# furio1999/EO_Diffusion

Measured on AMD Instinct MI355X. Metric: denoising steps/sec (UNet fwd + DDPM update) at 256x256 bs=16, higher is better.
Workload: dtype f32; 1 GPU; DDPM sampling step, 256x256x3, batch 16 per GPU, UNet arch A0 (base 128, mults [1,2,3,4], 1 res-block(s), attn_res []), Philox noise, x0-clipped update; global_batch=16, image_size=256, parallelism=batch-sharded x1, accumulate=fp32, precision_mode=fp32x3

## Files before the change

eo_diffusion_amd/csrc/igemm.hip:

```cpp
#include <type_traits>

#include "common.h"

struct IgemmP {
    const char* a0;
    const char* a1;
    const char* b;
    const float* bias;
    const float* cbias;
    const char* res;
    char* y;
    long long cbias_stride;
    int N, H, W, C0, C1, Cin, Cout, KS, stride, pad, ups, pad_tl, Ho, Wo, HoWo, Heff, Weff;
    int tw_log2, th;
    int tiles_pw, tiles_pi;
    long long lda, ldb, ldc, sa0, sa1, sb0, sb1, sc0, sc1;
    int nb1, bias_mode, c_f32;
    long long M;
    int Ncols, K, taps, KT, tiles_m, tiles_n, out_nchw;
    int kc0, kc1;
    int tapmajor_log2;
    int ldk;
    const float* gn_ss;
    int gn_silu;
// ... 1503 lines not shown
                for (int i = 0; i < TM; ++i)
#pragma unroll
                    for (int j = 0; j < TN; ++j)
                        acc[i][j] = DIRECT ? __builtin_amdgcn_mfma_f32_16x16x32_f16(__builtin_bit_cast(half8, bl[j]), __builtin_bit_cast(half8, ah[i]), acc[i][j], 0, 0, 0)
                                           : __builtin_amdgcn_mfma_f32_16x16x32_f16(__builtin_bit_cast(half8, ah[i]), __builtin_bit_cast(half8, bl[j]), acc[i][j], 0, 0, 0);
#pragma unroll
                for (int i = 0; i < TM; ++i)
#pragma unroll
                    for (int j = 0; j < TN; ++j)
                        acc[i][j] = DIRECT ? __builtin_amdgcn_mfma_f32_16x16x32_f16(__builtin_bit_cast(half8, bh[j]), __builtin_bit_cast(half8, ah[i]), acc[i][j], 0, 0, 0)
                                           : __builtin_amdgcn_mfma_f32_16x16x32_f16(__builtin_bit_cast(half8, ah[i]), __builtin_bit_cast(half8, bh[j]), acc[i][j], 0, 0, 0);
            } else {
#pragma unroll
                for (int s2 = 0; s2 < 2; ++s2) {
                    const int o = ((4 * s2 + lh) ^ bsw) * 16;
                    i32x4 fa16[TM], fb16[TN];
#pragma unroll
                    for (int i = 0; i < TM; ++i) fa16[i] = *reinterpret_cast<const i32x4*>(stg + a_rd + i * MS * BKB + o);
#pragma unroll
                    for (int j = 0; j < TN; ++j) fb16[j] = *reinterpret_cast<const i32x4*>(stg + b_rd2 + j * MS * BKB + o);
#pragma unroll
                    for (int i = 0; i < TM; ++i)
#pragma unroll
                        for (int j = 0; j < TN; ++j)
                            acc[i][j] = __builtin_amdgcn_mfma_f32_16x16x32_f16(__builtin_bit_cast(half8, fa16[i]), __builtin_bit_cast(half8, fb16[j]), acc[i][j], 0, 0, 0);
                }
            }
        }
      }
    }
    __builtin_amdgcn_s_waitcnt(0xc07f);
    __builtin_amdgcn_s_barrier();
    EOD_STAMP_AT(2);
    IgemmP pe = p;
    if constexpr (KSPLIT) pe.y = p.y + (long long)blockIdx.y * p.M * p.Cout * 4;
    if constexpr (SPLIT) {
        pe.alpha = p.alpha * wsc1 * asc.inv;
        if constexpr (DIRECT) halo_epilogue_direct<BM, BN, WAVES_M, WAVES_N>(pe, g, acc, wave, lane, n0, pre_bq, pe.alpha, pre_we);
        else igemm_epilogue<T, true, BM, BN, WAVES_M, WAVES_N, true, MS>(pe, g, acc, smem, wave, lane, n0, nullptr, 0, pre_bcol);
    } else if constexpr (sizeof(T) == 2) {
        igemm_epilogue<T, true, BM, BN, WAVES_M, WAVES_N, KSPLIT, MS>(pe, g, acc, smem, wave, lane, n0, nullptr, 0, pre_bcol);
    } else {
        igemm_epilogue<T, true, BM, BN, WAVES_M, WAVES_N, sizeof(T) == 4, MS>(pe, g, acc, smem, wave, lane, n0, nullptr, 0, pre_bcol);
    }
    }
    EOD_STAMP_AT(3);
}

template <typename T, bool SPLIT, bool BWD = false>
__global__ __launch_bounds__(256, 2) void conv_up4_halo_kernel(const IgemmP p) {
    static_assert(!SPLIT || sizeof(T) == 4, "the split-fp16 product is a mode of fp32 storage");
    static_assert(SPLIT || sizeof(T) == 2, "fp16 storage or split fp32");
    constexpr int NW = 4, WAVES_M = 2, WAVES_N = 2, BN = 128, BM = 128, MS = 16;
    constexpr int PH = 10, PW = 18, PR = PH * PW, PG = (PR + 7) / 8, LAH = (PG + NW - 1) / NW;
    constexpr int ES = sizeof(T), EPC = 16 / ES, BKB = 128, BK = BKB / ES;
    constexpr int WM = BM / WAVES_M, WN = BN / WAVES_N, TM = WM / MS, TN = WN / MS;
    constexpr int LB = (BN / 8) / NW;
    constexpr int ABUF = PG * 1024, BSTAGE = BN * BKB;
    static_assert(LAH == 6, "schedule: three patch pieces per K-step in steps 0 and 1");

    extern __shared__ __attribute__((aligned(16))) char smem[];
    char* const sA = smem;
    char* const sB = smem + 2 * ABUF;

    constexpr bool DIRECT = SPLIT && !BWD;
    const int tid = threadIdx.x, lane = tid & 63;
    const int wave = __builtin_amdgcn_readfirstlane(tid >> 6);
    const int wm = wave / WAVES_N, wn = wave % WAVES_N;
    int tile_m, tile_nn;
    map_tile(p, tile_m, tile_nn);
    const int tpc = BWD ? p.tiles_n : p.tiles_n >> 2;
    const int cls = BWD ? 0 : tile_nn / tpc, n0 = (tile_nn - cls * tpc) * BN;
    const int par_y = cls >> 1, par_x = cls & 1;
    const TileGeom g = make_geom<true, BM>(p, tile_m);
    float pre_bcol[DIRECT ? 1 : TN];
    f32x4 pre_bq[DIRECT ? TN : 1];
    int pre_we[DIRECT ? TN : 1];
    if constexpr (DIRECT) {
        prefetch_bcol4<TN>(p, p.Cout, n0 + wn * WN, lane, g.n_first, pre_bq);
        prefetch_wexp4<TN>(p, p.Cout, n0 + wn * WN, cls * p.Cout, lane, pre_we);
    } else {
        prefetch_bcol<TN, MS>(p, p.Cout, n0 + wn * WN, lane, g.n_first, pre_bcol);
    }
    float wsc1 = 1.0f;
    if constexpr (SPLIT) wsc1 = p.w_scale[1];
    AbScale asc = {EOD_SPLIT_ASCALE, 1.0f};
    if constexpr (SPLIT) {
        if (p.a_bound) asc = ab_scale_of(ab_wave_bound(p.a_bound, g.n_first));
    }

    const int srow = lane >> 3, sslot = lane & 7;
    unsigned ppix[LAH];
    const int bchunk0 = sslot ^ ((4 * wave + (srow >> 1)) & 7);
    unsigned pck = 0, pvalid = 0;
#pragma unroll
    for (int i = 0; i < LAH; ++i) {
        const int prow = (wave + NW * i) * 8 + srow;
        const int py = prow / PW, px = prow - py * PW;
        const int hi = g.ty0 - 1 + py, wi = g.tx0 - 1 + px;
        const bool ok = (wave + NW * i) < PG && prow < PR && (unsigned)hi < (unsigned)p.H && (unsigned)wi < (unsigned)p.W;
        if (ok) pvalid |= 1u << i;
        ppix[i] = BWD ? (unsigned)(4 * hi * p.W + 2 * wi)
                      : (unsigned)(hi * p.W + wi);
        pck |= (unsigned)(sslot ^ ((px >> 1) & 7)) << (3 * i);
    }
    auto pchunk_of = [&](int i) { return (int)((pck >> (3 * i)) & 7u); };
    unsigned b_v[LB];
#pragma unroll
    for (int i = 0; i < LB; ++i) {
        const int row = (wave + NW * i) * 8 + srow;
        b_v[i] = (n0 + row < p.Cout) ? (unsigned)(row * (BWD ? 4 * p.C0 : p.Cin) * ES) + bchunk0 * 16 : EOD_OOB;
    }
    const __amdgpu_buffer_rsrc_t rsA = make_rsrc(p.a0 + (long long)g.n_first * p.H * p.W * p.C0 * ES * (BWD ? 4 : 1));
    const int bpitch = BWD ? 4 * p.C0 : p.Cin;
    const __amdgpu_buffer_rsrc_t rsB = make_rsrc(p.b + ((long long)cls * p.Cout + n0) * bpitch * ES);
    const int tapstride = (BWD ? p.Cout * bpitch : 4 * p.Cout * p.Cin) * ES;

    struct Chunk {
        int kin, cls;
        bool ktail;
    };
    auto chunk_of = [&](int cc) {
        Chunk c;
        c.cls = BWD ? (cc & 3) : cls;
        c.kin = (BWD ? (cc >> 2) : cc) * BK;
        c.ktail = c.kin + BK > p.C0;
        return c;
    };
    auto issue_patch_piece = [&](int i, const Chunk& c, char* abuf) {
        const int pc = pchunk_of(i);
        unsigned v = ((pvalid >> i) & 1u) ? ppix[i] * (unsigned)(p.C0 * ES) + pc * 16 : EOD_OOB;
        if (c.ktail) v = (c.kin + pc * EPC < p.C0) ? v : EOD_OOB;
        const unsigned soff = (unsigned)(c.kin * ES) + (BWD ? (unsigned)(((c.cls >> 1) * 2 * p.W + (c.cls & 1)) * p.C0 * ES) : 0u);
        blds16(rsA, v, soff, abuf + (wave + NW * i) * 1024);
    };
    auto split_piece = [&](int i, char* abuf) {
        char* ptr = abuf + (wave + NW * i) * 1024 + lane * 16;
        const f32x4 f = *reinterpret_cast<const f32x4*>(ptr);
        *reinterpret_cast<i32x4*>(ptr) = split_pair_exchange_scaled(f, asc.s, (pchunk_of(i) & 1) != 0);
    };
    auto issue_weights = [&](int s, const Chunk& c, char* bst) {
        const int oy = BWD ? 1 - (c.cls >> 1) : par_y, ox = BWD ? 1 - (c.cls & 1) : par_x;
        const int tap = (oy + (s & 1)) * 3 + ox + (s >> 1);
        const unsigned soff = (unsigned)(tap * tapstride) + (unsigned)((c.kin + (BWD ? c.cls * p.C0 : 0)) * ES);
#pragma unroll
        for (int i = 0; i < LB; ++i) {
            unsigned v = b_v[i];
            if (c.ktail) v = (c.kin + (SPLIT ? (bchunk0 >> 1) * 8 : bchunk0 * EPC) < p.C0) ? v : EOD_OOB;
            blds16(rsB, v, soff, bst + (wave + NW * i) * 1024);
        }
    };
    auto wait_vm = [](int n) {
        switch (n) {
            case 0: asm volatile("s_waitcnt vmcnt(0)" ::: "memory"); break;
            case 1: asm volatile("s_waitcnt vmcnt(1)" ::: "memory"); break;
            case 2: asm volatile("s_waitcnt vmcnt(2)" ::: "memory"); break;
            case 3: asm volatile("s_waitcnt vmcnt(3)" ::: "memory"); break;
            case 4: asm volatile("s_waitcnt vmcnt(4)" ::: "memory"); break;
            case 5: asm volatile("s_waitcnt vmcnt(5)" ::: "memory"); break;
            default: asm volatile("s_waitcnt vmcnt(6)" ::: "memory"); break;
        }
    };

    typename AccLayout<MS>::vec acc[TM][TN];
#pragma unroll
    for (int i = 0; i < TM; ++i)
#pragma unroll
        for (int j = 0; j < TN; ++j)
#pragma unroll
            for (int r = 0; r < AccLayout<MS>::R; ++r) acc[i][j][r] = 0.0f;

    const int lr = lane & 15, lh = lane >> 4;
    const int c0 = SPLIT ? 2 * ((0x2130 >> (4 * lh)) & 3) : lh, c1 = SPLIT ? c0 + 1 : 4 + lh;
    int acur[2][2];
    auto set_acur = [&](int oy, int ox, int aoff) {
#pragma unroll
        for (int b = 0; b < 2; ++b) {
            const int pxc = lr + ox + b;
            const int key = (pxc >> 1) & 7;
            const int rowb = ((wm * (WM / 16) + oy) * PW + pxc) * BKB + aoff;
            acur[0][b] = rowb + ((c0 ^ key) << 4);
            acur[1][b] = rowb + ((c1 ^ key) << 4);
        }
    };
    set_acur(BWD ? 1 : par_y, BWD ? 1 : par_x, 0);
    const int bsw = (lr >> 1) & 7;
    const int b_rd = (wn * WN + lr) * BKB;
    const int boff0 = b_rd + ((c0 ^ bsw) << 4), boff1 = b_rd + ((c1 ^ bsw) << 4);

    i32x4 aw[2][TM];
    auto a_load = [&](int v, int b, int a) {
#pragma unroll
        for (int r = 0; r < TM + 1; ++r)
            if (a == 0 ? r < TM : r == TM) aw[v][r % TM] = *reinterpret_cast<const i32x4*>(sA + acur[v][b] + r * PW * BKB);
    };
    const int KC = BWD ? 4 * p.kc0 : p.kc0, NSTEP = KC * 4;
    {
        const Chunk ch0 = chunk_of(0);
#pragma unroll
        for (int i = 0; i < LAH; ++i)
            if ((wave + NW * i) < PG) issue_patch_piece(i, ch0, sA);
        issue_weights(0, ch0, sB);
        if constexpr (SPLIT) {
            asm volatile("s_waitcnt vmcnt(0)" ::: "memory");
#pragma unroll
            for (int i = 0; i < LAH; ++i)
                if ((wave + NW * i) < PG) split_piece(i, sA);
        }
    }
    int np_prev = 0;
    int step = 0;
    for (int cc = 0; cc < KC; ++cc) {
        const Chunk cur = chunk_of(cc);
        const bool has_next = cc + 1 < KC;
        const Chunk nxt = chunk_of(has_next ? cc + 1 : cc);
        char* abuf_next = sA + ((cc + 1) & 1) * ABUF;
#pragma unroll
        for (int s = 0; s < 4; ++s, ++step) {
            wait_vm(np_prev);
            if constexpr (SPLIT) __builtin_amdgcn_s_waitcnt(0xc07f);
            __builtin_amdgcn_s_barrier();
            const bool w_next = step + 1 < NSTEP;
            if (w_next) issue_weights((s + 1) & 3, s == 3 ? nxt : cur, sB + ((step + 1) & 1) * BSTAGE);
            int np = 0;
            if (s < 2 && has_next) {
#pragma unroll
                for (int k = 0; k < 3; ++k)
                    if ((wave + NW * (3 * s + k)) < PG) {
                        issue_patch_piece(3 * s + k, nxt, abuf_next);
                        ++np;
                    }
            }
            const int a = s & 1, b = s >> 1;
            const char* bst = sB + (step & 1) * BSTAGE;
            if constexpr (SPLIT) {
                i32x4 bh[TN], bl[TN];
                a_load(1, b, a);
#pragma unroll
                for (int j = 0; j < TN; ++j) bh[j] = *reinterpret_cast<const i32x4*>(bst + boff0 + j * MS * BKB);
                a_load(0, b, a);
#pragma unroll
                for (int i = 0; i < TM; ++i)
#pragma unroll
                    for (int j = 0; j < TN; ++j)
                        acc[i][j] = DIRECT ? __builtin_amdgcn_mfma_f32_16x16x32_f16(__builtin_bit_cast(half8, bh[j]), __builtin_bit_cast(half8, aw[1][(i + a) % TM]), acc[i][j], 0, 0, 0)
                                           : __builtin_amdgcn_mfma_f32_16x16x32_f16(__builtin_bit_cast(half8, aw[1][(i + a) % TM]), __builtin_bit_cast(half8, bh[j]), acc[i][j], 0, 0, 0);
#pragma unroll
                for (int j = 0; j < TN; ++j) bl[j] = *reinterpret_cast<const i32x4*>(bst + boff1 + j * MS * BKB);
#pragma unroll
                for (int i = 0; i < TM; ++i)
#pragma unroll
                    for (int j = 0; j < TN; ++j)
                        acc[i][j] = DIRECT ? __builtin_amdgcn_mfma_f32_16x16x32_f16(__builtin_bit_cast(half8, bl[j]), __builtin_bit_cast(half8, aw[0][(i + a) % TM]), acc[i][j], 0, 0, 0)
                                           : __builtin_amdgcn_mfma_f32_16x16x32_f16(__builtin_bit_cast(half8, aw[0][(i + a) % TM]), __builtin_bit_cast(half8, bl[j]), acc[i][j], 0, 0, 0);
#pragma unroll
                for (int i = 0; i < TM; ++i)
#pragma unroll
                    for (int j = 0; j < TN; ++j)
                        acc[i][j] = DIRECT ? __builtin_amdgcn_mfma_f32_16x16x32_f16(__builtin_bit_cast(half8, bh[j]), __builtin_bit_cast(half8, aw[0][(i + a) % TM]), acc[i][j], 0, 0, 0)
                                           : __builtin_amdgcn_mfma_f32_16x16x32_f16(__builtin_bit_cast(half8, aw[0][(i + a) % TM]), __builtin_bit_cast(half8, bh[j]), acc[i][j], 0, 0, 0);
            } else {
#pragma unroll
                for (int v = 0; v < 2; ++v) {
                    i32x4 fb16[TN];
                    a_load(v, b, a);
#pragma unroll
                    for (int j = 0; j < TN; ++j) fb16[j] = *reinterpret_cast<const i32x4*>(bst + (v ? boff1 : boff0) + j * MS * BKB);
#pragma unroll
                    for (int i = 0; i < TM; ++i)
#pragma unroll
                        for (int j = 0; j < TN; ++j)
                            acc[i][j] = __builtin_amdgcn_mfma_f32_16x16x32_f16(__builtin_bit_cast(half8, aw[v][(i + a) % TM]), __builtin_bit_cast(half8, fb16[j]), acc[i][j], 0, 0, 0);
                }
            }
            if constexpr (SPLIT) {
                if (s >= 2 && has_next) {
#pragma unroll
                    for (int k = 0; k < 3; ++k)
                        if ((wave + NW * (3 * (s - 2) + k)) < PG) split_piece(3 * (s - 2) + k, abuf_next);
                }
            }
            np_prev = np;
        }
        if constexpr (BWD) {
            const int ncl = (cc + 1) & 3;
            set_acur(1 - (ncl >> 1), 1 - (ncl & 1), ((cc + 1) & 1) * ABUF);
        } else {
            const int flip = (cc & 1) ? -ABUF : ABUF;
#pragma unroll
            for (int b = 0; b < 2; ++b) {
                acur[0][b] += flip;
                acur[1][b] += flip;
            }
        }
    }
    __builtin_amdgcn_s_waitcnt(0xc07f);
    __builtin_amdgcn_s_barrier();
    IgemmP pe = p;
    pe.Ncols = p.Cout;
    TileGeom ge = g;
    if constexpr (!BWD) {
        pe.par = 1; pe.par_y = par_y; pe.par_x = par_x;
        pe.Wd = p.W;
        pe.tiles_per_image = p.tiles_pi * 4;
        ge.tile_m = g.n_first * pe.tiles_per_image + (tile_m - g.n_first * p.tiles_pi) * 4 + cls;
    }
    if constexpr (SPLIT) pe.alpha = p.alpha * wsc1 * asc.inv;
    if constexpr (!BWD) pe.w_row0 = cls * p.Cout;
    if constexpr (DIRECT) halo_epilogue_direct<BM, BN, WAVES_M, WAVES_N>(pe, ge, acc, wave, lane, n0, pre_bq, pe.alpha, pre_we);
    else igemm_epilogue<T, true, BM, BN, WAVES_M, WAVES_N, sizeof(T) == 4, MS>(pe, ge, acc, smem, wave, lane, n0, nullptr, 0, pre_bcol);
}

template <typename T, bool SPLIT, bool BWD = false> static int launch_up4(IgemmP& p, hipStream_t st) {
    constexpr int BK = 128 / (int)sizeof(T);
    const size_t ring = 2 * (size_t)(23 * 1024) + 2 * (size_t)128 * 128;
    const size_t epi = 4 * (size_t)64 * (64 + 4) * sizeof(float);
    const size_t lds = ring > epi ? ring : epi;
    auto kern = conv_up4_halo_kernel<T, SPLIT, BWD>;
    static bool attr_done = false;
    if (!attr_done) {
        (void)hipFuncSetAttribute(reinterpret_cast<const void*>(kern), hipFuncAttributeMaxDynamicSharedMemorySize, (int)lds);
        attr_done = true;
    }
    p.kc0 = (p.C0 + BK - 1) / BK;
    p.kc1 = 0;
    p.KT = p.kc0 * 4;
    p.tiles_n = (BWD ? 1 : 4) * ((p.Cout + 127) / 128);
    p.tw_log2 = 4;
    p.th = 8;
    p.tiles_pw = (p.W + 15) / 16;
    p.tiles_pi = p.tiles_pw * (p.H / 8);
    p.tiles_m = p.tiles_pi * p.N;
    const long long nblk = (long long)p.tiles_m * p.tiles_n;
    if (nblk <= 0 || nblk > 0x7fffffffLL) {
        eod_set_error("conv_up4: bad grid %lld", nblk);
        return EOD_EINVAL;
    }
    hipLaunchKernelGGL(kern, dim3((unsigned)nblk), dim3(256), lds, st, p);
    EOD_CHECK_LAUNCH("conv_up4_halo");
    return EOD_OK;
}

template <typename T, bool SPLIT>
__global__ __launch_bounds__(256, 2) void conv_s2_halo_kernel(const IgemmP p) {
    static_assert(!SPLIT || sizeof(T) == 4, "the split-fp16 product is a mode of fp32 storage");
    static_assert(SPLIT || sizeof(T) == 2, "fp16 storage or split fp32");
    constexpr int NW = 4, WAVES_M = 2, WAVES_N = 2, BN = 128, BM = 128, MS = 16;
    constexpr int PH = 9, PW = 17, PR = PH * PW, PG = (PR + 7) / 8, LAH = (PG + NW - 1) / NW;
    constexpr int ES = sizeof(T), EPC = 16 / ES, BKB = 128, BK = BKB / ES;
    constexpr int WM = BM / WAVES_M, WN = BN / WAVES_N, TM = WM / MS, TN = WN / MS;
    constexpr int LB = (BN / 8) / NW;
    constexpr int ABUF = PG * 1024, BSTAGE = BN * BKB;
    static_assert(PG == NW * LAH && LAH * 4 <= 32, "every wave stages LAH whole pieces; 4 plane-validity bits per piece");
    static_assert(LB <= 6, "wait_vm immediates");

    extern __shared__ __attribute__((aligned(16))) char smem[];
    char* const sA = smem;
    char* const sB = smem + 2 * ABUF;

    constexpr bool DIRECT = SPLIT;
    const int tid = threadIdx.x, lane = tid & 63;
    const int wave = __builtin_amdgcn_readfirstlane(tid >> 6);
    const int wm = wave / WAVES_N, wn = wave % WAVES_N;
    int tile_m, tile_n;
    map_tile(p, tile_m, tile_n);
    const int n0 = tile_n * BN;
    const TileGeom g = make_geom<true, BM>(p, tile_m);
    float pre_bcol[DIRECT ? 1 : TN];
    f32x4 pre_bq[DIRECT ? TN : 1];
    int pre_we[DIRECT ? TN : 1];
    if constexpr (DIRECT) {
        prefetch_bcol4<TN>(p, p.Cout, n0 + wn * WN, lane, g.n_first, pre_bq);
        prefetch_wexp4<TN>(p, p.Cout, n0 + wn * WN, 0, lane, pre_we);
    } else {
        prefetch_bcol<TN, MS>(p, p.Cout, n0 + wn * WN, lane, g.n_first, pre_bcol);
    }
    float wsc1 = 1.0f;
    if constexpr (SPLIT) wsc1 = p.w_scale[1];
    AbScale asc = {EOD_SPLIT_ASCALE, 1.0f};
    if constexpr (SPLIT) {
        if (p.a_bound) asc = ab_scale_of(ab_wave_bound(p.a_bound, g.n_first));
    }

    const int srow = lane >> 3, sslot = lane & 7;
    int ppix[LAH];
    unsigned pvalid = 0, pck = 0;
    const int bchunk0 = sslot ^ ((4 * wave + (srow >> 1)) & 7);
#pragma unroll
    for (int i = 0; i < LAH; ++i) {
        const int prow = (wave + NW * i) * 8 + srow;
        const int py = prow / PW, px = prow - py * PW;
        const int hi = 2 * (g.ty0 + py) - 1, wi = 2 * (g.tx0 + px) - 1;
// ... 929 lines not shown
    if (tiles <= 0 || tiles >= 128 || kt < 8) return 1;
    int s = (int)(512 / tiles);
    if (s > kt / 4) s = kt / 4;
    if (s > 16) s = 16;
    return s < 2 ? 1 : s;
}

enum { FAM_UP4, FAM_UP4_BWD, FAM_FIRST, FAM_S2_HALO, FAM_HEAD, FAM_HALO, FAM_GENERIC, FAM_GENERIC_PARITY };
struct ConvPlan {
    int Heff, Weff, Ho, Wo;
    bool halo;
    int family;
    int bn;
    bool plus128;
    bool direct;
    int splitk, splitk_per;
    int tpw;
    int64_t workspace_bytes;
    int stats_slots;
    bool gn_fusable, skip_ok;
};
static ConvPlan conv_plan(const eod_conv_desc* d) {
    ConvPlan pl = {};
    pl.bn = 128;
    pl.splitk = pl.tpw = 1;
    if (d->upsample == 4) {
        pl.family = FAM_UP4_BWD;
        pl.Heff = pl.Ho = d->H / 2;
        pl.Weff = pl.Wo = d->W / 2;
        return pl;
    }
    pl.Heff = d->H * (d->upsample ? 2 : 1);
    pl.Weff = d->W * (d->upsample ? 2 : 1);
    const int Ho = pl.Ho = conv_out_hw(d, pl.Heff), Wo = pl.Wo = conv_out_hw(d, pl.Weff);
    const bool split = d->w_split, exact = !split && d->dtype != EOD_F16, gn = d->gn_scale_shift, skip = d->skip_x;
    pl.halo = conv_uses_halo(d, Ho, Wo);
    pl.splitk = conv_splitk(d, Ho, Wo, pl.halo, opt(OPT_HALO_SPLITK) != 0, &pl.splitk_per);
    pl.workspace_bytes = pl.splitk > 1 ? (int64_t)pl.splitk * d->N * Ho * Wo * d->Cout * 4 : 0;

    if (d->out_nchw_f32 || d->Cout % (16 / eod_esize(d->dtype))) pl.stats_slots = 0;
    else if (d->upsample == 3) pl.stats_slots = (d->H / 8) * ((d->W + 15) / 16) * 8;
    else if (pl.splitk > 1) pl.stats_slots = 1;
    else if (pl.halo) pl.stats_slots = (Ho / 8) * ((Wo + 15) / 16) * 2;
    else if ((Ho * Wo) % 128 != 0) pl.stats_slots = 0;
    else pl.stats_slots = (Ho * Wo / 128) * (d->Cout > 64 ? 2 : 4);

    const int max_cout = opt(OPT_GN_FUSE_MAX_COUT) >= 0 ? opt(OPT_GN_FUSE_MAX_COUT) : (split ? 512 : 256);
    pl.gn_fusable = !d->upsample && d->Cout <= max_cout && pl.halo;
    pl.skip_ok = opt(OPT_SKIP_FUSE) != 0 && conv_skip_geom_ok(d) && pl.halo;

    const long long tiles_pi = (long long)(Ho / 8) * ((Wo + 15) / 16);
    if (d->upsample == 3) {
        pl.family = FAM_UP4;
    } else if (opt(OPT_FIRST) != 0 && conv_first_ok(d, Ho, Wo)) {
        pl.family = FAM_FIRST;
    } else if (opt(OPT_S2_HALO) != 0 && conv_s2_halo_ok(d, Ho, Wo) && pl.splitk <= 1) {
        pl.family = FAM_S2_HALO;
    } else if (opt(OPT_HEAD) != 0 && pl.halo && conv_head_ok(d)) {
        pl.family = FAM_HEAD;
        int tpw = opt(OPT_HEAD_TPW);
        if (tpw <= 0) {
            tpw = 16;
            while (tpw > 1 && (tiles_pi % tpw || tiles_pi * d->N / tpw < 512)) tpw >>= 1;
        }
        while (tpw > 1 && tiles_pi % tpw) --tpw;
        pl.tpw = tpw;
    } else if (pl.halo) {
        pl.family = FAM_HALO;
        const bool on256 = opt(OPT_HALO_BN256) != 0;
        if (d->Cout <= 32) {
            pl.bn = 32;
        } else if (d->upsample || pl.splitk > 1) {
            pl.bn = 128;
        } else if (!exact && 16 * tiles_pi * ((d->Cout + 127) / 128) < 256) {
            pl.bn = 64;
        } else if (on256 && d->Cout % 256 == 0 && d->N * tiles_pi * (d->Cout / 256) >= 256 && ((gn && !exact) || (split && skip))) {
            pl.bn = 256;
        } else if (on256 && d->Cout > 256 && d->Cout % 256 == 128 && d->N * tiles_pi * ((d->Cout - 128) / 256) >= 256 && split && gn) {
            pl.bn = 256;
            pl.plus128 = true;
        }
    } else {
        pl.family = pl.splitk <= 1 && !split && conv_parity_ok(d, Ho, Wo) ? FAM_GENERIC_PARITY : FAM_GENERIC;
        pl.bn = generic_bn(d->Cout);
        if (split && d->Cout > 64) {
            const long long M = (long long)d->N * Ho * Wo;
            if (d->Cout % 256 == 0 && pl.splitk <= 1 && ((M + 127) / 128) * (d->Cout / 256) >= 256 && opt(OPT_HALO_BN256)) pl.bn = 256;
            pl.direct = pl.splitk <= 1 && !d->out_nchw_f32 && (Ho * Wo) % 128 == 0 && M % 128 == 0 && d->Cout % 4 == 0;
        }
    }
    return pl;
}

extern "C" int eod_conv_skip_ok(const eod_conv_desc* d) { return d && conv_plan(d).skip_ok ? 1 : 0; }
extern "C" int eod_conv_gn_fusable(const eod_conv_desc* d) { return d && conv_plan(d).gn_fusable ? 1 : 0; }
extern "C" int64_t eod_conv_workspace_size(const eod_conv_desc* d) { return d ? conv_plan(d).workspace_bytes : 0; }
extern "C" int eod_conv_stats_slots(const eod_conv_desc* d) { return d ? conv_plan(d).stats_slots : 0; }
extern "C" const char* eod_conv_kernel_name(const eod_conv_desc* d) {
    if (!d) return "";
    const ConvPlan pl = conv_plan(d);
    switch (pl.family) {
        case FAM_UP4: case FAM_UP4_BWD: return "conv_up4_halo_kernel";
        case FAM_FIRST: return "conv_first_x3_kernel";
        case FAM_S2_HALO: return "conv_s2_halo_kernel";
        case FAM_HEAD: return "conv_head_kernel";
        case FAM_HALO: return pl.bn == 32 ? "conv3x3_halo_kernel<BN=32>" : "conv3x3_halo_kernel";
        default: return "igemm_kernel";
    }
}

extern "C" int eod_conv_halo_columns(const eod_conv_desc* d) {
    if (!d) return 0;
    const ConvPlan pl = conv_plan(d);
    return pl.family == FAM_HALO ? pl.bn : 0;
}

static int conv_up4_bwd(const eod_conv_desc* d, void* stream) {
    EOD_REQUIRE(d->N > 0 && d->H > 0 && d->W > 0 && d->C0 > 0 && d->Cout > 0 && d->x && d->w && d->y, "conv (upsample 4): bad args");
    EOD_REQUIRE(conv_up4_bwd_ok(d), "conv: upsample = 4 needs a geometry for which eod_conv_up4_bwd_ok(d) == 1");
    EOD_REQUIRE(eod_aligned16(d->x) && eod_aligned16(d->w), "conv: 16-byte alignment");
    EOD_REQUIRE((long long)d->H * d->W * d->C0 * 2 < 0x7fffffffLL && 9LL * d->Cout * 4 * d->C0 * 2 < 0x7fffffffLL, "conv (upsample 4): operand exceeds the 2 GiB window");
    const ConvPlan pl = conv_plan(d);
    IgemmP p = {};
    p.a0 = (const char*)d->x; p.b = (const char*)d->w; p.bias = d->bias; p.bias_mode = d->bias ? 1 : 0;
    p.cbias = d->cbias; p.cbias_stride = d->cbias_stride; p.res = (const char*)d->res; p.y = (char*)d->y;
    p.N = d->N; p.H = pl.Ho; p.W = pl.Wo;
    p.C0 = d->C0; p.C1 = 0; p.Cin = d->C0; p.Cout = d->Cout; p.KS = 3; p.stride = 1; p.pad = 1;
    p.Ho = pl.Ho; p.Wo = pl.Wo; p.HoWo = pl.Ho * pl.Wo; p.Heff = pl.Heff; p.Weff = pl.Weff;
    p.Hd = pl.Ho; p.Wd = pl.Wo; p.HWd = pl.Ho * pl.Wo;
    p.M = (long long)d->N * pl.Ho * pl.Wo; p.Ncols = d->Cout; p.taps = 9; p.alpha = d->alpha; p.nb1 = 1; p.tapmajor_log2 = -1;
    return launch_up4<half_t, false, true>(p, (hipStream_t)stream);
}

static IgemmP splitk_partial(const IgemmP& p, const eod_conv_desc* d, const ConvPlan& pl) {
    IgemmP q = p;
    q.stats = nullptr;
    q.splitk = pl.splitk;
    q.splitk_per = pl.splitk_per;
    q.y = (char*)d->workspace;
    q.bias = nullptr; q.bias_mode = 0; q.cbias = nullptr; q.res = nullptr; q.alpha = 1.0f;
    return q;
}
static int splitk_finish(const eod_conv_desc* d, const IgemmP& p, int splitk, hipStream_t st) {
    if (d->stats) {
        const dim3 grid((unsigned)((p.Cout + 63) / 64), (unsigned)d->N);
        if (d->dtype == EOD_F16)
            hipLaunchKernelGGL(splitk_reduce_stats_kernel<half_t>, grid, dim3(256), 0, st, (const float*)d->workspace, splitk, p.M, p.Cout, p.HoWo, d->alpha, d->bias, d->cbias, (long long)d->cbias_stride, (const half_t*)d->res, (half_t*)d->y, d->stats);
        else
            hipLaunchKernelGGL(splitk_reduce_stats_kernel<float>, grid, dim3(256), 0, st, (const float*)d->workspace, splitk, p.M, p.Cout, p.HoWo, d->alpha, d->bias, d->cbias, (long long)d->cbias_stride, (const float*)d->res, (float*)d->y, d->stats);
        EOD_CHECK_LAUNCH("splitk_reduce_stats");
        return EOD_OK;
    }
    const long long total4 = p.M * p.Cout / 4;
    const unsigned blocks = (unsigned)((total4 + 255) / 256 > 2048 ? 2048 : (total4 + 255) / 256);
    if (d->dtype == EOD_F16)
        hipLaunchKernelGGL(splitk_reduce_kernel<half_t>, dim3(blocks), dim3(256), 0, st, (const float*)d->workspace, splitk, p.M, p.Cout, p.HoWo, d->alpha, d->bias, d->cbias, (long long)d->cbias_stride, (const half_t*)d->res, (half_t*)d->y, (const float*)nullptr);
    else
        hipLaunchKernelGGL(splitk_reduce_kernel<float>, dim3(blocks), dim3(256), 0, st, (const float*)d->workspace, splitk, p.M, p.Cout, p.HoWo, d->alpha, d->bias, d->cbias, (long long)d->cbias_stride, (const float*)d->res, (float*)d->y, (const float*)nullptr);
    EOD_CHECK_LAUNCH("splitk_reduce");
    return EOD_OK;
}
static int conv_require_workspace(const eod_conv_desc* d, const ConvPlan& pl) {
    EOD_REQUIRE(d->workspace && d->workspace_bytes >= pl.workspace_bytes, "conv: workspace of %lld bytes required (eod_conv_workspace_size)", (long long)pl.workspace_bytes);
    return EOD_OK;
}

template <typename T, bool SPLIT, int MS, bool GN, bool SKIP>
// ... 55 lines not shown
    IgemmP p = {};
    p.a0 = (const char*)d->x;
    p.a1 = (const char*)d->x2;
    p.b = (const char*)d->w;
    p.bias = d->bias;
    p.bias_mode = d->bias ? 1 : 0;
    p.cbias = d->cbias;
    p.cbias_stride = d->cbias_stride;
    p.res = (const char*)d->res;
    p.y = (char*)d->y;
    p.N = d->N; p.H = d->H; p.W = d->W; p.C0 = d->C0; p.C1 = d->C1; p.Cin = d->C0 + d->C1; p.Cout = d->Cout;
    p.KS = d->ksize; p.stride = d->stride; p.pad = d->pad; p.ups = d->upsample; p.pad_tl = d->pad_tl;
    p.Ho = Ho; p.Wo = Wo; p.HoWo = Ho * Wo; p.Heff = pl.Heff; p.Weff = pl.Weff;
    p.Hd = Ho; p.Wd = Wo; p.HWd = Ho * Wo;
    p.M = (long long)d->N * Ho * Wo;
    p.Ncols = d->Cout;
    p.taps = d->ksize * d->ksize;
    p.out_nchw = d->out_nchw_f32;
    p.alpha = d->alpha;
    p.nb1 = 1;
    p.tapmajor_log2 = -1;
    if (d->w_tapmajor) {
        const int cpt = d->C0 / epc;
        EOD_REQUIRE(d->ksize == 3 && d->C1 == 0 && !d->upsample && !d->pad_tl && !d->gn_scale_shift && (cpt == 1 || cpt == 2 || cpt == 4),
                    "conv: w_tapmajor needs a 3x3 conv of a single source with C0 in {1,2,4} x %d channels", epc);
        p.tapmajor_log2 = cpt == 1 ? 0 : cpt == 2 ? 1 : 2;
        p.ldk = eod_conv_tapmajor_ldk(d->C0, d->dtype);
    }
    hipStream_t st = (hipStream_t)stream;
    if (d->stats) {
        EOD_REQUIRE(pl.stats_slots > 0 && pl.stats_slots == d->stats_slots, "conv: stats_slots=%d but this geometry provides %d", d->stats_slots, pl.stats_slots);
        p.stats = d->stats;
        p.stats_P = pl.stats_slots;
        p.tiles_per_image = Ho * Wo / 128;
    }
    EOD_REQUIRE(!d->w_split || (conv_split_ok(d) && d->w_scale),
                "conv: w_split needs a geometry for which eod_conv_split_ok(d) == 1 and the w_scale of eod_pack_conv_weight_split");
    p.w_scale = d->w_split ? d->w_scale : nullptr;
    p.w_rexp = d->w_split ? reinterpret_cast<const int*>(d->w_scale) + 4 : nullptr;
    p.w_row0 = 0;
    p.a_bound = d->w_split ? d->a_bound : nullptr;
    EOD_REQUIRE(!d->x_presplit || (d->w_split && d->a_bound && !pl.halo && !d->upsample && !d->w_tapmajor && !d->gn_scale_shift),
                "conv: x_presplit needs w_split with the producer's bound table, on the generic kernel (1x1 / stride-2 / small maps)");
    p.a_ps = d->x_presplit;
    EOD_REQUIRE(!d->y_presplit_bound || (d->w_split && !pl.halo && !d->out_nchw_f32 && !d->stats && d->Cout % 8 == 0 && (Ho * Wo) % 128 == 0 &&
                                         pl.splitk <= 1),
                "conv: y_presplit_bound needs w_split on the generic kernel, Cout %% 8 == 0, whole 128-row tiles per image, no statistics");
    p.y_ps_bound = d->y_presplit_bound;
    p.skip_bound = (d->w_split && d->skip_x) ? d->skip_bound : nullptr;
    const bool f16 = d->dtype == EOD_F16;
    switch (pl.family) {
        case FAM_UP4:
            EOD_REQUIRE(conv_up4_ok(d), "conv: upsample = 3 (parity-class form of the nearest-2x conv) needs a geometry for which eod_conv_up4_ok(d) == 1");
            return f16 ? launch_up4<half_t, false>(p, st) : launch_up4<float, true>(p, st);
        case FAM_FIRST: return d->C0 == 4 ? launch_first<4>(p, st) : launch_first<8>(p, st);
        case FAM_S2_HALO: return f16 ? launch_s2<half_t, false>(p, st) : launch_s2<float, true>(p, st);
        case FAM_HEAD:
            p.gn_ss = d->gn_scale_shift;
            p.gn_silu = d->gn_silu;
            p.tpw = pl.tpw;
            return f16 ? launch_head<half_t, false>(p, st) : launch_head<float, true>(p, st);
        default: break;
    }
    const bool splitk = pl.splitk > 1;
    if (pl.family == FAM_HALO && splitk) {
        const int rc = conv_require_workspace(d, pl);
        if (rc != EOD_OK) return rc;
    }
    if (d->skip_x) {
        EOD_REQUIRE(pl.skip_ok && d->skip_w, "conv: skip_x needs a geometry for which eod_conv_skip_ok(d) == 1, and skip_w");
        EOD_REQUIRE((d->skip_C1 > 0) == (d->skip_x2 != nullptr), "conv: skip_x2 / skip_C1 mismatch");
        EOD_REQUIRE(eod_aligned16(d->skip_x) && eod_aligned16(d->skip_x2) && eod_aligned16(d->skip_w), "conv: 16-byte alignment (skip operands)");
        const long long smax = d->skip_C0 > d->skip_C1 ? d->skip_C0 : d->skip_C1;
        EOD_REQUIRE((long long)d->H * d->W * smax * es < 0x7fffffffLL && (long long)d->Cout * (d->skip_C0 + d->skip_C1) * es < 0x7fffffffLL,
                    "conv: skip operand exceeds the 2 GiB window");
        p.sx0 = (const char*)d->skip_x;
        p.sx1 = (const char*)d->skip_x2;
        p.b2 = (const char*)d->skip_w;
        p.SC0 = d->skip_C0;
        p.SC1 = d->skip_C1;
    }
    if (pl.family == FAM_HALO) {
        if (d->gn_scale_shift) {
            EOD_REQUIRE(!d->upsample, "conv: fused input GroupNorm is not available together with upsample");
            p.gn_ss = d->gn_scale_shift;
            p.gn_silu = d->gn_silu;
        }
        IgemmP q = splitk ? splitk_partial(p, d, pl) : p;
        const int rc = d->w_split ? launch_halo_T<float, true, 16>(q, d, pl, st)
                                  : f16 ? launch_halo_T<half_t, false, 16>(q, d, pl, st) : launch_halo_T<float, false, 32>(q, d, pl, st);
        return splitk && rc == EOD_OK ? splitk_finish(d, p, pl.splitk, st) : rc;
    }
    EOD_REQUIRE(!d->gn_scale_shift, "conv: fused input GroupNorm needs the halo-patch kernel (ask eod_conv_gn_fusable first)");
    if (pl.family == FAM_GENERIC_PARITY) {
        p.par = 1;
        p.Hd = Ho / 2; p.Wd = Wo / 2; p.HWd = p.Hd * p.Wd;
        p.M = (long long)d->N * p.HWd;
        for (int cls = 0; cls < 4; ++cls) {
            IgemmP q = p;
            q.par_y = cls >> 1; q.par_x = cls & 1;
            const int ndy = q.par_y ? 2 : 1, ndx = q.par_x ? 2 : 1;
            const int dys[2] = {q.par_y ? 0 : 1, 2}, dxs[2] = {q.par_x ? 0 : 1, 2};
            q.taps = 0; q.taplist = 0;
            for (int a = 0; a < ndy; ++a)
                for (int b = 0; b < ndx; ++b) q.taplist |= (unsigned)(dys[a] * 3 + dxs[b]) << (4 * q.taps++);
            const int rc = f16 ? launch_T<half_t, true>(q, 1, st) : launch_T<float, true>(q, 1, st);
// ... 57 lines not shown
```

Measured before the change: 41.79 steps/s.

## Add 8-wave BN=256 upsample conv kernel and shrink parity-class patch window

Adds an 8-wave, 256-column variant of the parity-class nearest-2x upsample conv for the split-fp16 fp32 path. It is selected when the grid stays large enough, with a 128-column remainder handled by the existing kernel through a new n_base offset. It also shrinks the staged input patch from 10x18 to 9x17 in the forward path by folding the parity offset into the load coordinates. The aim is to reuse each staged input patch across more output channels and to load less halo. The cost is higher LDS and register use at one block per CU, plus possibly two launches per conv.

After: 42.23 steps/s, median of 6. +1.1%, better.

```diff
diff --git a/eo_diffusion_amd/csrc/igemm.hip b/eo_diffusion_amd/csrc/igemm.hip
--- a/eo_diffusion_amd/csrc/igemm.hip
+++ b/eo_diffusion_amd/csrc/igemm.hip
@@ -1579,12 +1579,13 @@
     static_assert(!SPLIT || sizeof(T) == 4, "the split-fp16 product is a mode of fp32 storage");
     static_assert(SPLIT || sizeof(T) == 2, "fp16 storage or split fp32");
     constexpr int NW = 4, WAVES_M = 2, WAVES_N = 2, BN = 128, BM = 128, MS = 16;
-    constexpr int PH = 10, PW = 18, PR = PH * PW, PG = (PR + 7) / 8, LAH = (PG + NW - 1) / NW;
+    constexpr int PH = BWD ? 10 : 9, PW = BWD ? 18 : 17, PR = PH * PW, PG = (PR + 7) / 8, LAH = (PG + NW - 1) / NW;
     constexpr int ES = sizeof(T), EPC = 16 / ES, BKB = 128, BK = BKB / ES;
     constexpr int WM = BM / WAVES_M, WN = BN / WAVES_N, TM = WM / MS, TN = WN / MS;
     constexpr int LB = (BN / 8) / NW;
     constexpr int ABUF = PG * 1024, BSTAGE = BN * BKB;
-    static_assert(LAH == 6, "schedule: three patch pieces per K-step in steps 0 and 1");
+    static_assert(LAH == (BWD ? 6 : 5), "schedule: up to three patch pieces per K-step in steps 0 and 1");
+    static_assert((WAVES_M - 1) * (WM / 16) + TM + (BWD ? 1 : 0) < PH && 15 + 1 + (BWD ? 1 : 0) < PW, "the fragment reads stay inside the staged patch");
 
     extern __shared__ __attribute__((aligned(16))) char smem[];
     char* const sA = smem;
@@ -1597,7 +1598,7 @@
     int tile_m, tile_nn;
     map_tile(p, tile_m, tile_nn);
     const int tpc = BWD ? p.tiles_n : p.tiles_n >> 2;
-    const int cls = BWD ? 0 : tile_nn / tpc, n0 = (tile_nn - cls * tpc) * BN;
+    const int cls = BWD ? 0 : tile_nn / tpc, n0 = (BWD ? 0 : p.n_base) + (tile_nn - cls * tpc) * BN;
     const int par_y = cls >> 1, par_x = cls & 1;
     const TileGeom g = make_geom<true, BM>(p, tile_m);
     float pre_bcol[DIRECT ? 1 : TN];
@@ -1624,7 +1625,7 @@
     for (int i = 0; i < LAH; ++i) {
         const int prow = (wave + NW * i) * 8 + srow;
         const int py = prow / PW, px = prow - py * PW;
-        const int hi = g.ty0 - 1 + py, wi = g.tx0 - 1 + px;
+        const int hi = g.ty0 - 1 + py + (BWD ? 0 : par_y), wi = g.tx0 - 1 + px + (BWD ? 0 : par_x);
         const bool ok = (wave + NW * i) < PG && prow < PR && (unsigned)hi < (unsigned)p.H && (unsigned)wi < (unsigned)p.W;
         if (ok) pvalid |= 1u << i;
         ppix[i] = BWD ? (unsigned)(4 * hi * p.W + 2 * wi)
@@ -1710,7 +1711,7 @@
             acur[1][b] = rowb + ((c1 ^ key) << 4);
         }
     };
-    set_acur(BWD ? 1 : par_y, BWD ? 1 : par_x, 0);
+    set_acur(BWD ? 1 : 0, BWD ? 1 : 0, 0);
     const int bsw = (lr >> 1) & 7;
     const int b_rd = (wn * WN + lr) * BKB;
     const int boff0 = b_rd + ((c0 ^ bsw) << 4), boff1 = b_rd + ((c1 ^ bsw) << 4);
@@ -1753,7 +1754,7 @@
             if (s < 2 && has_next) {
 #pragma unroll
                 for (int k = 0; k < 3; ++k)
-                    if ((wave + NW * (3 * s + k)) < PG) {
+                    if (3 * s + k < LAH && (wave + NW * (3 * s + k)) < PG) {
                         issue_patch_piece(3 * s + k, nxt, abuf_next);
                         ++np;
                     }
@@ -1804,7 +1805,7 @@
                 if (s >= 2 && has_next) {
 #pragma unroll
                     for (int k = 0; k < 3; ++k)
-                        if ((wave + NW * (3 * (s - 2) + k)) < PG) split_piece(3 * (s - 2) + k, abuf_next);
+                        if (3 * (s - 2) + k < LAH && (wave + NW * (3 * (s - 2) + k)) < PG) split_piece(3 * (s - 2) + k, abuf_next);
                 }
             }
             np_prev = np;
@@ -1840,7 +1841,7 @@
 
 template <typename T, bool SPLIT, bool BWD = false> static int launch_up4(IgemmP& p, hipStream_t st) {
     constexpr int BK = 128 / (int)sizeof(T);
-    const size_t ring = 2 * (size_t)(23 * 1024) + 2 * (size_t)128 * 128;
+    const size_t ring = 2 * (size_t)((BWD ? 23 : 20) * 1024) + 2 * (size_t)128 * 128;
     const size_t epi = 4 * (size_t)64 * (64 + 4) * sizeof(float);
     const size_t lds = ring > epi ? ring : epi;
     auto kern = conv_up4_halo_kernel<T, SPLIT, BWD>;
@@ -1852,7 +1853,7 @@
     p.kc0 = (p.C0 + BK - 1) / BK;
     p.kc1 = 0;
     p.KT = p.kc0 * 4;
-    p.tiles_n = (BWD ? 1 : 4) * ((p.Cout + 127) / 128);
+    p.tiles_n = BWD ? (p.Cout + 127) / 128 : 4 * ((p.Cout - p.n_base + 127) / 128);
     p.tw_log2 = 4;
     p.th = 8;
     p.tiles_pw = (p.W + 15) / 16;
@@ -1865,6 +1866,230 @@
     }
     hipLaunchKernelGGL(kern, dim3((unsigned)nblk), dim3(256), lds, st, p);
     EOD_CHECK_LAUNCH("conv_up4_halo");
+    return EOD_OK;
+}
+
+template <typename T, bool SPLIT, bool BWD, int WAVES_N>
+__global__ __launch_bounds__(512, 1) void conv_up4_halo_kernel(const IgemmP p) {
+    static_assert(SPLIT && !BWD && sizeof(T) == 4 && WAVES_N == 4, "the 8-wave form: forward, split product of fp32 storage");
+    constexpr int NW = 8, WAVES_M = 2, RW = 4, BN = 256, BM = 128, MS = 16;
+    constexpr int PH = 9, PW = 17, PR = PH * PW, PG = (PR + 7) / 8, LAH = (PG + RW - 1) / RW;
+    constexpr int ES = sizeof(T), EPC = 16 / ES, BKB = 128, BK = BKB / ES;
+    constexpr int WM = BM / WAVES_M, WN = BN / WAVES_N, TM = WM / MS, TN = WN / MS;
+    constexpr int LBR = (BN / 8) / RW;
+    constexpr int ABUF = PG * 1024, BSTAGE = BN * BKB;
+    constexpr bool EARLY = true;
+    static_assert(LAH == 5 && PG == RW * LAH && LBR % 2 == 0, "schedule: 3 + 2 patch pieces, every wave holds all five; the prologue halves the weight pieces");
+    static_assert((WAVES_M - 1) * (WM / 16) + TM < PH && 15 + 1 < PW, "the fragment reads stay inside the staged window");
+
+    extern __shared__ __attribute__((aligned(16))) char smem[];
+    char* const sA = smem;
+    char* const sB = smem + 2 * ABUF;
+
+    const int tid = threadIdx.x, lane = tid & 63;
+    const int wave = __builtin_amdgcn_readfirstlane(tid >> 6);
+    const int wm = wave / WAVES_N, wn = wave % WAVES_N;
+    const int wr = wn;
+    int tile_m, tile_nn;
+    map_tile(p, tile_m, tile_nn);
+    const int tpc = p.tiles_n >> 2;
+    const int cls = tile_nn / tpc, n0 = (tile_nn - cls * tpc) * BN;
+    const int par_y = cls >> 1, par_x = cls & 1;
+    const TileGeom g = make_geom<true, BM>(p, tile_m);
+    f32x4 pre_bq[TN];
+    int pre_we[TN];
+    prefetch_bcol4<TN>(p, p.Ncols, n0 + wn * WN, lane, g.n_first, pre_bq);
+    prefetch_wexp4<TN>(p, p.Ncols, n0 + wn * WN, cls * p.Cout, lane, pre_we);
+    const float wsc1 = p.w_scale[1];
+    AbScale asc = {EOD_SPLIT_ASCALE, 1.0f};
+    if (p.a_bound) asc = ab_scale_of(ab_wave_bound(p.a_bound, g.n_first));
+
+    const int srow = lane >> 3, sslot = lane & 7;
+    unsigned ppix[LAH];
+    const int bchunk0 = sslot ^ ((4 * wave + (srow >> 1)) & 7);
+    unsigned pck = 0, pvalid = 0;
+#pragma unroll
+    for (int i = 0; i < LAH; ++i) {
+        const int prow = (wr + RW * i) * 8 + srow;
+        const int py = prow / PW, px = prow - py * PW;
+        const int hi = g.ty0 - 1 + py + par_y, wi = g.tx0 - 1 + px + par_x;
+        const bool ok = prow < PR && (unsigned)hi < (unsigned)p.H && (unsigned)wi < (unsigned)p.W;
+        if (ok) pvalid |= 1u << i;
+        ppix[i] = (unsigned)(hi * p.W + wi);
+        pck |= (unsigned)(sslot ^ ((px >> 1) & 7)) << (3 * i);
+    }
+    auto pchunk_of = [&](int i) { return (int)((pck >> (3 * i)) & 7u); };
+    const int brem = p.Ncols - n0 - (wr * 8 + srow);
+    const unsigned b_v = (unsigned)((wr * 8 + srow) * p.Cin * ES) + bchunk0 * 16;
+    const __amdgpu_buffer_rsrc_t rsA = make_rsrc(p.a0 + (long long)g.n_first * p.H * p.W * p.C0 * ES);
+    const __amdgpu_buffer_rsrc_t rsB = make_rsrc(p.b + ((long long)cls * p.Cout + n0) * p.Cin * ES);
+    const int tapstride = 4 * p.Cout * p.Cin * ES;
+
+    struct Chunk {
+        int kin;
+        bool ktail;
+    };
+    auto chunk_of = [&](int cc) {
+        Chunk c;
+        c.kin = cc * BK;
+        c.ktail = c.kin + BK > p.C0;
+        return c;
+    };
+    auto issue_patch_piece = [&](int i, const Chunk& c, char* abuf) {
+        const int pc = pchunk_of(i);
+        unsigned v = ((pvalid >> i) & 1u) ? ppix[i] * (unsigned)(p.C0 * ES) + pc * 16 : EOD_OOB;
+        if (c.ktail) v = (c.kin + pc * EPC < p.C0) ? v : EOD_OOB;
+        blds16(rsA, v, (unsigned)(c.kin * ES), abuf + (wr + RW * i) * 1024);
+    };
+    auto split_piece = [&](int i, char* abuf) {
+        char* ptr = abuf + (wr + RW * i) * 1024 + lane * 16;
+        const f32x4 f = *reinterpret_cast<const f32x4*>(ptr);
+        *reinterpret_cast<i32x4*>(ptr) = split_pair_exchange_scaled(f, asc.s, (pchunk_of(i) & 1) != 0);
+    };
+    auto issue_weight_tile = [&](int s, const Chunk& c, char* bst, int i0, int i1) {
+        const int tap = (par_y + (s & 1)) * 3 + par_x + (s >> 1);
+        const unsigned soff = (unsigned)(tap * tapstride) + (unsigned)(c.kin * ES);
+        unsigned v = b_v;
+        if (c.ktail) v = (c.kin + (bchunk0 >> 1) * 8 < p.C0) ? v : EOD_OOB;
+#pragma unroll
+        for (int i = 0; i < LBR; ++i)
+            if (i >= i0 && i < i1) blds16(rsB, brem > RW * 8 * i ? v : EOD_OOB, soff + (unsigned)(RW * 8 * i * p.Cin * ES), bst + (wr + RW * i) * 1024);
+    };
+
+    f32x4 acc[TM][TN];
+#pragma unroll
+    for (int i = 0; i < TM; ++i)
+#pragma unroll
+        for (int j = 0; j < TN; ++j) acc[i][j] = f32x4{0.0f, 0.0f, 0.0f, 0.0f};
+
+    const int lr = lane & 15, lh = lane >> 4;
+    const int c0 = 2 * ((0x2130 >> (4 * lh)) & 3), c1 = c0 + 1;
+    int acur[2][2];
+#pragma unroll
+    for (int b = 0; b < 2; ++b) {
+        const int pxc = lr + b;
+        const int key = (pxc >> 1) & 7;
+        const int rowb = (wm * (WM / 16) * PW + pxc) * BKB;
+        acur[0][b] = rowb + ((c0 ^ key) << 4);
+        acur[1][b] = rowb + ((c1 ^ key) << 4);
+    }
+    const int bsw = (lr >> 1) & 7;
+    const int b_rd = (wn * WN + lr) * BKB;
+    const int boff0 = b_rd + ((c0 ^ bsw) << 4), boff1 = b_rd + ((c1 ^ bsw) << 4);
+    i32x4 aw[2][TM];
+    auto a_load = [&](int v, int b, int a) {
+#pragma unroll
+        for (int r = 0; r < TM + 1; ++r)
+            if (a == 0 ? r < TM : r == TM) aw[v][r % TM] = *reinterpret_cast<const i32x4*>(sA + acur[v][b] + r * PW * BKB);
+    };
+    const int KC = p.kc0, NSTEP = KC * 4;
+    {
+        const Chunk ch0 = chunk_of(0);
+#pragma unroll
+        for (int i = 0; i < LAH; ++i)
+            if ((i >= 3) == (wm != 0)) issue_patch_piece(i, ch0, sA);
+        issue_weight_tile(0, ch0, sB, wm * (LBR / 2), (wm + 1) * (LBR / 2));
+        asm volatile("s_waitcnt vmcnt(0)" ::: "memory");
+#pragma unroll
+        for (int i = 0; i < LAH; ++i)
+            if ((i >= 3) == (wm != 0)) split_piece(i, sA);
+    }
+    int step = 0;
+    for (int cc = 0; cc < KC; ++cc) {
+        const Chunk cur = chunk_of(cc);
+        const bool has_next = cc + 1 < KC;
+        const Chunk nxt = chunk_of(has_next ? cc + 1 : cc);
+        char* abuf_next = sA + ((cc + 1) & 1) * ABUF;
+#pragma unroll
+        for (int s = 0; s < 4; ++s, ++step) {
+            if (wm == 1) asm volatile("s_waitcnt vmcnt(0)" ::: "memory");
+            __builtin_amdgcn_s_waitcnt(0xc07f);
+            __builtin_amdgcn_s_barrier();
+            if (wm == 1 && step + 1 < NSTEP) issue_weight_tile((s + 1) & 3, s == 3 ? nxt : cur, sB + ((step + 1) & 1) * BSTAGE, 0, LBR);
+            const int a = s & 1, b = s >> 1;
+            const char* bst = sB + (step & 1) * BSTAGE;
+            const bool a_here = !EARLY || s == 0, a_early = EARLY && s < 3;
+            const int na = (s + 1) & 1, nb = (s + 1) >> 1;
+            i32x4 bh[TN], bl[TN];
+            if (a_here) a_load(1, b, a);
+#pragma unroll
+            for (int j = 0; j < TN; ++j) bh[j] = *reinterpret_cast<const i32x4*>(bst + boff0 + j * MS * BKB);
+            if (a_here) a_load(0, b, a);
+#pragma unroll
+            for (int i = 0; i < TM; ++i)
+#pragma unroll
+                for (int j = 0; j < TN; ++j)
+                    acc[i][j] = __builtin_amdgcn_mfma_f32_16x16x32_f16(__builtin_bit_cast(half8, bh[j]), __builtin_bit_cast(half8, aw[1][(i + a) % TM]), acc[i][j], 0, 0, 0);
+#pragma unroll
+            for (int j = 0; j < TN; ++j) bl[j] = *reinterpret_cast<const i32x4*>(bst + boff1 + j * MS * BKB);
+            if (a_early) a_load(1, nb, na);
+#pragma unroll
+            for (int i = 0; i < TM; ++i)
+#pragma unroll
+                for (int j = 0; j < TN; ++j)
+                    acc[i][j] = __builtin_amdgcn_mfma_f32_16x16x32_f16(__builtin_bit_cast(half8, bl[j]), __builtin_bit_cast(half8, aw[0][(i + a) % TM]), acc[i][j], 0, 0, 0);
+#pragma unroll
+            for (int i = 0; i < TM; ++i)
+#pragma unroll
+                for (int j = 0; j < TN; ++j)
+                    acc[i][j] = __builtin_amdgcn_mfma_f32_16x16x32_f16(__builtin_bit_cast(half8, bh[j]), __builtin_bit_cast(half8, aw[0][(i + a) % TM]), acc[i][j], 0, 0, 0);
+            if (a_early) a_load(0, nb, na);
+            if (wm == 0 && has_next) {
+                if (s < 2) {
+#pragma unroll
+                    for (int k = 0; k < 3; ++k)
+                        if (3 * s + k < LAH) issue_patch_piece(3 * s + k, nxt, abuf_next);
+                } else {
+                    if (s == 2) asm volatile("s_waitcnt vmcnt(2)" ::: "memory");
+                    else asm volatile("s_waitcnt vmcnt(0)" ::: "memory");
+#pragma unroll
+                    for (int k = 0; k < 3; ++k)
+                        if (3 * (s - 2) + k < LAH) split_piece(3 * (s - 2) + k, abuf_next);
+                }
+            }
+        }
+        const int flip = (cc & 1) ? -ABUF : ABUF;
+#pragma unroll
+        for (int b = 0; b < 2; ++b) {
+            acur[0][b] += flip;
+            acur[1][b] += flip;
+        }
+    }
+    IgemmP pe = p;
+    TileGeom ge = g;
+    pe.par = 1; pe.par_y = par_y; pe.par_x = par_x;
+    pe.Wd = p.W;
+    pe.tiles_per_image = p.tiles_pi * 4;
+    ge.tile_m = g.n_first * pe.tiles_per_image + (tile_m - g.n_first * p.tiles_pi) * 4 + cls;
+    pe.alpha = p.alpha * wsc1 * asc.inv;
+    pe.w_row0 = cls * p.Cout;
+    halo_epilogue_direct<BM, BN, WAVES_M, WAVES_N>(pe, ge, acc, wave, lane, n0, pre_bq, pe.alpha, pre_we);
+}
+
+static int launch_up4_w8(IgemmP& p, hipStream_t st) {
+    const size_t lds = 2 * (size_t)(20 * 1024) + 2 * (size_t)256 * 128;
+    auto kern = conv_up4_halo_kernel<float, true, false, 4>;
+    static bool attr_done = false;
+    if (!attr_done) {
+        (void)hipFuncSetAttribute(reinterpret_cast<const void*>(kern), hipFuncAttributeMaxDynamicSharedMemorySize, (int)lds);
+        attr_done = true;
+    }
+    p.kc0 = (p.C0 + 31) / 32;
+    p.kc1 = 0;
+    p.KT = p.kc0 * 4;
+    p.tiles_n = 4 * ((p.Ncols + 255) / 256);
+    p.tw_log2 = 4;
+    p.th = 8;
+    p.tiles_pw = (p.W + 15) / 16;
+    p.tiles_pi = p.tiles_pw * (p.H / 8);
+    p.tiles_m = p.tiles_pi * p.N;
+    const long long nblk = (long long)p.tiles_m * p.tiles_n;
+    if (p.Ncols <= 0 || p.Ncols % 256 || nblk <= 0 || nblk > 0x7fffffffLL) {
+        eod_set_error("conv_up4 (8 waves): bad grid %lld, %d columns", nblk, p.Ncols);
+        return EOD_EINVAL;
+    }
+    hipLaunchKernelGGL(kern, dim3((unsigned)nblk), dim3(512), lds, st, p);
+    EOD_CHECK_LAUNCH("conv_up4_halo (8 waves)");
     return EOD_OK;
 }
 
@@ -2900,6 +3125,15 @@
     const long long tiles_pi = (long long)(Ho / 8) * ((Wo + 15) / 16);
     if (d->upsample == 3) {
         pl.family = FAM_UP4;
+        const long long wg = (long long)d->N * (d->H / 8) * ((d->W + 15) / 16) * 4;
+        if (split && d->dtype == EOD_F32 && opt(OPT_HALO_BN256) != 0 && conv_up4_ok(d)) {
+            if (d->Cout % 256 == 0 && wg * (d->Cout / 256) >= 256) {
+                pl.bn = 256;
+            } else if (d->Cout > 256 && d->Cout % 256 == 128 && wg * ((d->Cout - 128) / 256) >= 256) {
+                pl.bn = 256;
+                pl.plus128 = true;
+            }
+        }
     } else if (opt(OPT_FIRST) != 0 && conv_first_ok(d, Ho, Wo)) {
         pl.family = FAM_FIRST;
     } else if (opt(OPT_S2_HALO) != 0 && conv_s2_halo_ok(d, Ho, Wo) && pl.splitk <= 1) {
@@ -2960,7 +3194,7 @@
 extern "C" int eod_conv_halo_columns(const eod_conv_desc* d) {
     if (!d) return 0;
     const ConvPlan pl = conv_plan(d);
-    return pl.family == FAM_HALO ? pl.bn : 0;
+    return pl.family == FAM_HALO || pl.family == FAM_UP4 ? pl.bn : 0;
 }
 
 static int conv_up4_bwd(const eod_conv_desc* d, void* stream) {
@@ -3122,6 +3356,17 @@
     switch (pl.family) {
         case FAM_UP4:
             EOD_REQUIRE(conv_up4_ok(d), "conv: upsample = 3 (parity-class form of the nearest-2x conv) needs a geometry for which eod_conv_up4_ok(d) == 1");
+            if (pl.bn == 256) {
+                if (pl.plus128) {
+                    IgemmP q = p;
+                    q.Ncols = d->Cout - 128;
+                    const int rc = launch_up4_w8(q, st);
+                    if (rc != EOD_OK) return rc;
+                    p.n_base = d->Cout - 128;
+                    return launch_up4<float, true>(p, st);
+                }
+                return launch_up4_w8(p, st);
+            }
             return f16 ? launch_up4<half_t, false>(p, st) : launch_up4<float, true>(p, st);
         case FAM_FIRST: return d->C0 == 4 ? launch_first<4>(p, st) : launch_first<8>(p, st);
         case FAM_S2_HALO: return f16 ? launch_s2<half_t, false>(p, st) : launch_s2<float, true>(p, st);
```
